# genome-vendor/allpathslg

Measured on NVIDIA B200. Metric: k-mer spectrum throughput (K=25), k-mer instances counted per second, higher is better.
Workload: dtype u64

## Files before the change

allpathslg_b200/csrc/local3.cuh:

```cuda
#pragma once
#include "local2.cuh"

#ifndef L3_PREFETCH
#define L3_PREFETCH 1
#endif
namespace apgk {

constexpr int L3_ROW = 16;
constexpr int L3_SLACK = 96;
constexpr int L3_STACK = 72;

struct Local3Smem {
  uint32_t* key; uint32_t* cnt; uint32_t* bitmap; uint16_t* list; uint32_t* spec; uint32_t* wsum; uint32_t* misc;
  uint32_t* stack;
  static __host__ __device__ size_t slots(int LM) { return (((size_t)LM + LM / 4 + 1 + L3_SLACK) + 127) & ~(size_t)127; }
  __device__ __forceinline__ void carve(unsigned char* raw, int LM) {
    const size_t ns = slots(LM);
    key = (uint32_t*)raw;
    cnt = key + ns;
    bitmap = cnt + ns;
    spec = bitmap + ns / 32 + 4;
    wsum = spec + SPEC_SMEM;
    misc = wsum + 40;
    stack = misc + 8;
    list = (uint16_t*)(stack + 2 * L3_STACK);
  }
  static size_t bytes(int LM) {
    return (slots(LM) * 2 + slots(LM) / 32 + 4 + SPEC_SMEM + 40 + 8 + 2 * L3_STACK) * 4 + ((size_t)LM + LM / 4 + 128) * 2 + 16;
  }
};

template <int NT, int W>
__global__ void __launch_bounds__(NT, 1536 / NT) k_local3(const uint32_t* __restrict__ src, BucketTable bt, int rem_bits, EmitCtx<W> ec,
                                               uint32_t* __restrict__ nd_out) {
  extern __shared__ __align__(16) unsigned char smem_raw[];
  Local3Smem sm;
  const int LM = (int)bt.local_max;
  sm.carve(smem_raw, LM);
  const int tid = threadIdx.x, lane = tid & 31, wid = tid >> 5;
  constexpr int NWARP = NT / 32;
  for (int i = tid; i < SPEC_SMEM; i += NT) sm.spec[i] = 0;
  const int up = 32 - rem_bits;
  const uint32_t m_cap = (uint32_t)LM + (uint32_t)LM / 4 + 1;
  unsigned long long n_nx = 0, o_nx = 0;
  if (bt.b0 + blockIdx.x < bt.nb) { n_nx = bt.bsize[bt.b0 + blockIdx.x]; o_nx = bt.bofs[bt.b0 + blockIdx.x]; }
  for (uint32_t b = bt.b0 + blockIdx.x; b < bt.nb; b += gridDim.x) {
    const unsigned long long n64 = n_nx;
    const unsigned long long o = o_nx;
    {
      const uint32_t bn = b + gridDim.x;
      if (bn < bt.nb) { n_nx = bt.bsize[bn]; o_nx = bt.bofs[bn]; }
    }
    if (n64 == 0) {
      if (tid == 0) nd_out[b] = 0;
      continue;
    }
    const uint32_t* s = src + o;
    const uint32_t m_want = n64 < (unsigned long long)LM ? (uint32_t)n64 + ((uint32_t)n64 >> 2) + 1 : m_cap;
    const uint32_t nrows = (m_want + L3_ROW - 1) / L3_ROW;
    const uint32_t ns = nrows * L3_ROW;
    const uint32_t ns4 = (ns + 3) >> 2;
    const uint32_t nwords = (ns + 31) >> 5;
    volatile uint32_t* vmisc = sm.misc;
    uint32_t run_nd = 0;
    bool first = true;
    while (true) {
      __syncthreads();
      uint32_t sp = 1, rd = 0, ri = 0;
      if (!first) {
        sp = sm.misc[1];
        if (sp == 0) break;
        rd = sm.stack[2 * (sp - 1)];
        ri = sm.stack[2 * (sp - 1) + 1];
      }
      first = false;
      {
        uint4* k4 = reinterpret_cast<uint4*>(sm.key);
        uint4* c4 = reinterpret_cast<uint4*>(sm.cnt);
        const uint4 e4 = make_uint4(SLOT_EMPTY, SLOT_EMPTY, SLOT_EMPTY, SLOT_EMPTY), z4 = make_uint4(0, 0, 0, 0);
        for (uint32_t i = tid; i < ns4; i += NT) { k4[i] = e4; c4[i] = z4; }
        for (uint32_t i = tid; i < nwords + 2; i += NT) sm.bitmap[i] = 0;
        if (tid == 0) sm.misc[0] = 0;
      }
      __syncthreads();
      if (tid == 0) sm.misc[1] = sp - 1;
      const uint32_t pshift = 32 - rd;
      for (unsigned long long i0 = 0; i0 < n64; i0 += 4ull * NT) {
        uint32_t kk[4];
#pragma unroll
        for (int u = 0; u < 4; u++) {
          const unsigned long long i = i0 + (unsigned long long)u * NT + tid;
          kk[u] = i < n64 ? s[i] : SLOT_EMPTY;
        }
#pragma unroll
        for (int u = 0; u < 4; u++) {
          const uint32_t k = kk[u];
          const uint32_t x = k << up;
          if (k != SLOT_EMPTY && (rd == 0 || (x >> pshift) == ri)) {
            const uint32_t row = __umulhi(x << rd, nrows) * L3_ROW;
            uint32_t h = (k * 0x9E3779B1u) >> 28;
            uint32_t slot = row + h;
            uint32_t cur = atomicCAS(&sm.key[slot], SLOT_EMPTY, k);
            if (cur == SLOT_EMPTY) atomicOr(&sm.bitmap[slot >> 5], 1u << (slot & 31));
            bool placed = (cur == SLOT_EMPTY) | (cur == k);
            for (int pr = 1; !placed; pr++) {
              if (pr == L3_ROW) { sm.misc[0] = 1u; break; }
              h = (h + 1) & (L3_ROW - 1);
              slot = row + h;
              cur = atomicCAS(&sm.key[slot], SLOT_EMPTY, k);
              if (cur == SLOT_EMPTY) atomicOr(&sm.bitmap[slot >> 5], 1u << (slot & 31));
              placed = (cur == SLOT_EMPTY) | (cur == k);
            }
            if (placed) atomicAdd(&sm.cnt[slot], 1u);
          }
          __syncwarp();
        }
        if (n64 > (unsigned long long)LM && __any_sync(0xffffffffu, vmisc[0] != 0)) break;
      }
      __syncthreads();
#if L3_PREFETCH
      if (L3_PREFETCH == 1 || run_nd == 0) {
        const unsigned long long i = (unsigned long long)tid * 32;
        if (b + gridDim.x < bt.nb && i < n_nx && tid < 1024) prefetch_l2(src + o_nx + i);
      }
#endif
      uint32_t nd_total;
      {
        constexpr int WPT = 2;
        uint32_t wd[WPT], c = 0;
#pragma unroll
        for (int u = 0; u < WPT; u++) {
          const uint32_t wi = tid * WPT + u;
          wd[u] = wi < nwords ? sm.bitmap[wi] : 0u;
          c += __popc(wd[u]);
        }
        const uint32_t incl = warp_incl_scan(c, lane);
        if (lane == 31) sm.wsum[wid] = incl;
        __syncthreads();
        uint32_t base = incl - c;
        nd_total = 0;
#pragma unroll
        for (int w = 0; w < NWARP; w++) {
          const uint32_t v = sm.wsum[w];
          if (w < wid) base += v;
          nd_total += v;
        }
        const bool failed = sm.misc[0] != 0;
        if (!failed) {
#pragma unroll
          for (int u = 0; u < WPT; u++) {
            uint32_t w = wd[u];
            const uint32_t s_base = (tid * WPT + u) << 5;
            while (w) {
              const int bit = __ffs((int)w) - 1;
              w &= w - 1;
              sm.list[base++] = (uint16_t)(s_base + bit);
            }
          }
        }
      }
      __syncthreads();
      if (sm.misc[0] != 0) {
        if (tid == 0) {
          uint32_t top = sm.misc[1];
          if ((int)rd < rem_bits && top + 2 <= L3_STACK) {
            sm.stack[2 * top] = rd + 1; sm.stack[2 * top + 1] = 2 * ri + 1; top++;
            sm.stack[2 * top] = rd + 1; sm.stack[2 * top + 1] = 2 * ri; top++;
            sm.misc[1] = top;
          } else {
            sm.misc[2] = 1u;
          }
        }
        continue;
      }
      for (uint32_t j0 = 0; j0 < nd_total; j0 += NT) {
        const uint32_t j = j0 + tid;
        uint32_t f = 0;
        if (j < nd_total) {
          const uint32_t q = sm.list[j];
          const uint32_t k = sm.key[q];
          const uint32_t rbase = q & ~(uint32_t)(L3_ROW - 1);
          uint32_t rowbits = (sm.bitmap[q >> 5] >> (rbase & 31)) & 0xFFFFu;
          const uint32_t before = __popc(rowbits & ((1u << (q & (L3_ROW - 1))) - 1u));
          uint32_t smaller = 0;
          while (rowbits) {
            const int bit = __ffs((int)rowbits) - 1;
            rowbits &= rowbits - 1;
            smaller += sm.key[rbase + bit] < k;
          }
          const unsigned long long pos = o + run_nd + (j - before + smaller);
          f = sm.cnt[q];
          if (ec.want_table) {
            ec.tmp_keys[pos] = rebuild_key<W>(k, (uint64_t)b, ec.rem_bits, ec.pad);
            ec.tmp_cnt[pos] = f;
          }
        }
        const uint32_t ones = __ballot_sync(0xffffffffu, f == 1u);
        if (lane == 0 && ones) atomicAdd(&sm.spec[1], (uint32_t)__popc(ones));
        if (f > 1u) {
          if (f < SPEC_SMEM) atomicAdd(&sm.spec[f], 1u);
          else spec_add_global(ec.spec_dense, ec.spec_ovf, ec.spec_ovf_cap, f);
        }
      }
      run_nd += nd_total;
      if (sm.misc[1] == 0) break;
    }
    if (tid == 0) nd_out[b] = run_nd;
  }
  __syncthreads();
  for (int i = tid; i < SPEC_SMEM; i += NT) {
    const uint32_t v = sm.spec[i];
    if (v) atomicAdd(&ec.spec_dense[i], (unsigned long long)v);
  }
}

}
```

allpathslg_b200/csrc/apgk.cu:

```cuda
#include <algorithm>
#include <array>
#include <cmath>
#include <cstdio>
#include <cstdlib>
#include <cstring>
#include <ctime>
#include <map>
#include <string>
#include <type_traits>
#include <utility>
#include <vector>

#include "../../include/apgk.h"
#include "gfreq.cuh"

using namespace apgk;

namespace {

enum Stage { ST_HIST0, ST_SCAN0, ST_SCATTER0, ST_HIST1, ST_SCAN1, ST_SCATTER1, ST_LOCAL, ST_BIG, ST_TABLE, ST_SPECTRUM,
             ST_OWNER, ST_TOTAL, ST_PLAN, ST_REDUCE };
const char* kStageNames[APGK_N_STAGES] = {"hist0", "scan0", "scatter0", "hist1", "scan1", "scatter1",
                                          "local", "big", "table", "spectrum", "owner", "total", "plan", "reduce"};

// ... 136 lines not shown
    c->ivs.push_back(iv);
  }
  apgk_ctx::StageIv& iv = c->ivs[c->n_ivs];
  iv.stage = s; iv.ended = false;
  c->open_iv[s] = (int)c->n_ivs++;
  if (kTrace) fprintf(stderr, "[apgk %.2f] begin %s\n", trace_now(), kStageNames[s]);
  cudaEventRecord(iv.e0, c->stream);
}
void stage_end(apgk_ctx* c, int s) {
  const int i = c->open_iv[s];
  if (i < 0) return;
  cudaEventRecord(c->ivs[i].e1, c->stream);
  c->ivs[i].ended = true;
  c->open_iv[s] = -1;
  if (kTrace) fprintf(stderr, "[apgk %.2f] end   %s\n", trace_now(), kStageNames[s]);
}
void stages_collect(apgk_ctx* c) {
  for (size_t i = 0; i < c->n_ivs; i++) {
    float ms = 0;
    if (c->ivs[i].ended && cudaEventElapsedTime(&ms, c->ivs[i].e0, c->ivs[i].e1) == cudaSuccess) c->stage_ms[c->ivs[i].stage] += ms;
  }
  c->n_ivs = 0;
}

int words_for(int K) { return (2 * K + 63) / 64; }

template <int W> struct Geo;
#ifndef APGK_NT
#define APGK_NT 1024
#endif
template <> struct Geo<1> { static constexpr int NTS = APGK_NT; static constexpr int NPOS = 16; static constexpr int NT0 = APGK_NT; static constexpr int NT1 = APGK_NT; static constexpr uint32_t TILE1 = APGK_NT * 16; static constexpr int LM_KEY = 4096; };
template <> struct Geo<2> { static constexpr int NTS = 1024; static constexpr int NPOS = 8; static constexpr int NT0 = 512; static constexpr int NT1 = 512; static constexpr uint32_t TILE1 = 512 * 8;  static constexpr int LM_KEY = 2048; };
template <> struct Geo<3> { static constexpr int NTS = 1024; static constexpr int NPOS = 4; static constexpr int NT0 = 256; static constexpr int NT1 = 512; static constexpr uint32_t TILE1 = 512 * 5;  static constexpr int LM_KEY = 2048; };
constexpr int LM_U32 = 5120;
constexpr int LM_KEY4 = 3072;
static bool use_local4(int W) {
  static const bool off = getenv("APGK_NO_LOCAL4") != nullptr;
  static const bool all = getenv("APGK_LOCAL4") != nullptr && !strcmp(getenv("APGK_LOCAL4"), "all");
  return !off && (W == 1 || all);
}
constexpr int L3_NT = 512;
constexpr int COL_NT = 1024;

void build_plan(HostPlan& hp, const std::vector<uint64_t>& seg_sizes, uint32_t tile_elems, int bins) {
  const int S = (int)seg_sizes.size();
  hp.seg_tile0.assign(S + 1, 0); hp.seg_chunk0.assign(S + 1, 0); hp.seg_start.assign(S + 1, 0);
  uint64_t max_tiles = 1;
  for (int s = 0; s < S; s++) {
    uint64_t t = (seg_sizes[s] + tile_elems - 1) / tile_elems;
    hp.seg_tile0[s + 1] = hp.seg_tile0[s] + (uint32_t)t;
    hp.seg_start[s + 1] = hp.seg_start[s] + seg_sizes[s];
    max_tiles = std::max(max_tiles, t);
  }
  int ct = (int)((max_tiles + 3) / 4);
  ct = std::max(8, std::min(ct, 128));
  if (const char* e = getenv("APGK_CT")) { if (atoi(e) > 0) ct = atoi(e); }
  for (int s = 0; s < S; s++) {
    uint32_t t = hp.seg_tile0[s + 1] - hp.seg_tile0[s];
    hp.seg_chunk0[s + 1] = hp.seg_chunk0[s] + (t + ct - 1) / ct;
  }
  hp.lp.bins = bins; hp.lp.n_segments = S; hp.lp.chunk_tiles = ct;
  hp.lp.n_tiles = hp.seg_tile0[S]; hp.lp.n_chunks = hp.seg_chunk0[S]; hp.lp.tile_elems = tile_elems;
}

int column_scan(apgk_ctx* c, const HostPlan& hp, int fold, unsigned long long* bofs_out) {
  const LevelPlan& lp = hp.lp;
  if (lp.n_chunks == 0) return APGK_OK;
  CU(c->segtot.ensure((size_t)lp.n_segments * lp.bins * 8));
  CU(c->bstart32.ensure((size_t)lp.n_segments * lp.bins * 4));
  k_segscan<COL_NT><<<lp.n_segments, COL_NT, 0, c->stream>>>(lp, c->chunksum.as<uint32_t>(),
                                                            c->segtot.as<unsigned long long>(),
                                                            c->bstart32.as<uint32_t>(), bofs_out, fold);
  LAUNCHED();
  return APGK_OK;
// ... 86 lines not shown
    const uint64_t sb_byte = src_bit0 >> 3;
    const uint64_t sb_al = sb_byte & ~7ull;
    const size_t nbytes = (size_t)(((src_bit0 + 2 * n_bases + 7) >> 3) - sb_al);
    CU(c->staging.ensure(nbytes + 32));
    CU(cudaMemsetAsync((uint8_t*)c->staging.p + (nbytes & ~(size_t)7), 0, 24, c->stream));
    CU(cudaMemcpyAsync(c->staging.p, packed + sb_al, nbytes, cudaMemcpyHostToDevice, c->stream));
    const uint64_t nbits = 2 * n_bases;
    const uint64_t nwords = ((dst_bit0 + nbits + 63) >> 6) - (dst_bit0 >> 6);
    k_append_bits<<<(unsigned)((nwords + 255) / 256), 256, 0, c->stream>>>(
        c->staging.as<uint64_t>(), src_bit0 - sb_al * 8, c->bases.as<uint64_t>(), dst_bit0, nbits);
    LAUNCHED();
  }
  return APGK_OK;
}

void invalidate_results(apgk_ctx* c) {
  c->finished = false; c->have_table = false; c->spec_loaded = false;
  c->table_from_reads = false; c->have_occ = false; c->n_occ = 0;
  c->n_instances = c->n_distinct = 0;
  c->owner_ranks = 0;
  c->part_ready = false; c->part_n = 0;
}

enum RunMode { RUN_FULL = 0, RUN_PARTITION = 1 };
template <int W, typename ElemB>
int run_levels(apgk_ctx* c, const Key<W>* dev_keys, uint64_t n_keys, RunMode mode);
template <int W, typename ElemB>
int count_buckets(apgk_ctx* c, uint64_t Nr, uint64_t N_all, uint64_t& n_prev, Key<W>* tmp_keys, bool nosync);

uint64_t window_upper(const apgk_ctx* c) { return c->n_windows; }

template <int W>
bool select_geometry(apgk_ctx* c, uint64_t upper, int forced_P) {
  int lm_u32 = LM_U32;
  if (const char* e = getenv("APGK_LM")) { if (atoi(e) >= 256 && atoi(e) <= 12288) lm_u32 = atoi(e); }
  if (upper == 0) upper = 1;
  if (forced_P > 0) {
    make_geom(c, std::max(2, std::min(24, forced_P)));
    return W == 1 && c->geom.REM <= 32;
  }
  int P = choose_prefix_bits(c, upper, lm_u32, true);
  make_geom(c, P);
  if (W == 1 && c->cfg.prefix_bits <= 0 && !getenv("APGK_PREFIX_BITS")) {
    while (c->geom.REM > 31 && c->geom.REM <= 34 && P < 24) make_geom(c, ++P);
  }
  const bool u32 = (W == 1 && c->geom.REM <= 32);
  if (!u32) {
    P = use_local4(W) ? choose_prefix_bits(c, upper, LM_KEY4 * 3 / 4, true) : choose_prefix_bits(c, upper, Geo<W>::LM_KEY, false);
    make_geom(c, P);
  }
  return u32;
}

template <int W> int compact_table(apgk_ctx* c, uint64_t total);

enum { RES_RANGE_N = 0, RES_SUM_TOT0 = 1, RES_FLAGS = 2, RES_DISTINCT = 3, RES_TABLE_OVF = 4, RES_XFLAGS = 5, RES_WORDS = 16 };

int fetch_results(apgk_ctx* c) {
  CU(cudaMemcpyAsync(c->res_host, c->res.p, RES_WORDS * 8, cudaMemcpyDeviceToHost, c->stream));
  CU(cudaStreamSynchronize(c->stream));
  return APGK_OK;
}

int step_epilogue(apgk_ctx* c, bool full) {
  { int r2 = fetch_results(c); if (r2) return r2; }
  if (c->res_host[RES_FLAGS] & 1ull) FAIL(APGK_E_RANGE, "a level-0 bucket holds 2^32 or more k-mers");
  if (c->res_host[RES_SUM_TOT0] && c->res_host[RES_SUM_TOT0] != c->n_windows_run)
    FAIL(APGK_E_STATE, "internal: level-0 histogram counts %llu k-mers, the input holds %llu",
         (unsigned long long)c->res_host[RES_SUM_TOT0], (unsigned long long)c->n_windows_run);
  if (full && c->table_pending) {
    c->table_pending = false;
    const uint64_t total = c->res_host[RES_DISTINCT];
    if (c->res_host[RES_TABLE_OVF]) {
      int rc = APGK_E_ARG;
// ... 252 lines not shown
    const char* eb = getenv("APGK_BULK");
    const bool bulk = eb && !strcmp(eb, "1");
    const size_t smb = scatter_bulk_smem_bytes<ElemB>(tile, bins1);
    if (bulk && sizeof(ElemB) == 4 && smb <= 200 * 1024 && bins1 <= Geo<W>::NT1) {
      auto kern = k_scatter_keys_bulk<Key<W>, ElemB, Geo<W>::NT1, DIGIT_BITS, false>;
      { int rc = kernel_setup(c, kern, Geo<W>::NT1, smb, nullptr); if (rc) return rc; }
      kern<<<chunks_bound, Geo<W>::NT1, smb, c->stream>>>(a_src, lp, dg1, c->chunksum.as<uint32_t>(), nullptr, g.pad, g.REM,
                                                          c->B.as<ElemB>());
    } else {
      auto kern = ScatterSel<ElemB, W>::kernel();
      const size_t sm = scatter_smem_bytes<Key<W>>(tile, bins1);
      { int rc = kernel_setup(c, kern, Geo<W>::NT1, sm, nullptr); if (rc) return rc; }
      kern<<<chunks_bound, Geo<W>::NT1, sm, c->stream>>>(a_src, lp, dg1, c->chunksum.as<uint32_t>(), nullptr, g.pad, g.REM,
                                                         c->B.as<ElemB>());
    }
    LAUNCHED();
  }
  stage_end(c, ST_SCATTER1);
  return APGK_OK;
}

int temp_budget(apgk_ctx* c, size_t* budget) {
  size_t fr = 0, tot = 0;
  CU(cudaMemGetInfo(&fr, &tot));
  const size_t held = c->A.cap + c->B.cap + c->T.cap;
  *budget = (size_t)((double)(fr + held) * 0.60);
  return APGK_OK;
}

template <int W, typename ElemB>
int run_levels(apgk_ctx* c, const Key<W>* dev_keys, uint64_t n_keys, RunMode mode) {
  const KeyGeom g = c->geom;
  const int bins0 = 1 << g.D0, bins1 = 1 << g.D1;
  int local_max = std::is_same<ElemB, uint32_t>::value ? LM_U32 : (use_local4(W) ? LM_KEY4 : Geo<W>::LM_KEY);
  if (std::is_same<ElemB, uint32_t>::value) {
    if (const char* e = getenv("APGK_LM")) { if (atoi(e) >= 256 && atoi(e) <= 12288) local_max = atoi(e); }
  }
  const int want_table = (c->cfg.flags & APGK_WANT_COUNTS) ? 1 : 0;
  c->elem_bytes = sizeof(ElemB);
  c->local_max = (uint32_t)local_max;
  c->nb1 = (uint32_t)bins0 * (uint32_t)bins1;
  c->n_rounds = 0; c->n_big = 0; c->n_distinct = 0;
  c->table_pending = false;
  CU(c->spec_dense.ensure((size_t)SPEC_DENSE * 8));
  CU(cudaMemsetAsync(c->spec_dense.p, 0, (size_t)SPEC_DENSE * 8, c->stream));
  CU(c->out_off.ensure(((size_t)c->nb1 + 1) * 8));
  CU(cudaMemsetAsync(c->out_off.p, 0, ((size_t)c->nb1 + 1) * 8, c->stream));
  const uint64_t N = dev_keys ? n_keys : c->n_windows;
  c->n_instances = N; c->n_windows_run = N;
  c->tot0_host.assign((size_t)bins0, 0);
  if (N == 0) {
    { int rc = wait_ingest(c); if (rc) return rc; }
    c->have_table = want_table != 0;
    c->part_n = 0;
    if (mode == RUN_PARTITION) {
      CU(c->segtot.ensure((size_t)c->nb1 * 8));
      CU(cudaMemsetAsync(c->segtot.p, 0, (size_t)c->nb1 * 8, c->stream));
    }
    return APGK_OK;
  }

  DigitSpec ds0{DIGIT_BITS, g.TB - g.D0, g.D0, g.pad, 0};
  DigitFn<DIGIT_BITS> dg0 = make_digit_fn<DIGIT_BITS>(ds0);
  { int rc = level0_hist<W>(c, dev_keys, n_keys, dg0); if (rc) return rc; }

  const size_t eA = sizeof(Key<W>), eB = sizeof(ElemB) + (want_table ? 4 : 0);
  uint64_t cap_outer = c->cfg.max_round_keys, cap_inner = c->cfg.max_inner_keys;
  if (const char* e = getenv("APGK_ROUND_KEYS")) { if (atoll(e) > 0) cap_outer = (uint64_t)atoll(e); }
  if (const char* e = getenv("APGK_INNER_KEYS")) { if (atoll(e) > 0) cap_inner = (uint64_t)atoll(e); }
  bool single;
// ... 91 lines not shown
      { int rc = level1<W, ElemB>(c, (int)in[0], (int)in[1], n_in, a_src, 0); if (rc) return rc; }
      if (mode == RUN_PARTITION) { c->part_n = n_in; return APGK_OK; }
      c->count_src = c->B.p; c->bucket_lo = c->bucket_hi = 0;
      if (!single) { c->bucket_lo = (uint32_t)in[0] * (uint32_t)bins1; c->bucket_hi = (uint32_t)in[1] * (uint32_t)bins1; }
      c->table_scale = single ? 1.0 : std::max(1.0, (double)N / (double)std::max<uint64_t>(n_counted, 1));
      { int rc = count_buckets<W, ElemB>(c, n_in, N, n_prev, a_src, single); if (rc) return rc; }
      c->table_scale = 1.0;
      c->bucket_lo = c->bucket_hi = 0;
      off_a += n_in;
    }
  }
  if (!single) c->n_distinct = n_prev;
  c->have_table = want_table != 0;
  return APGK_OK;
}

template <int W>
int compact_table(apgk_ctx* c, uint64_t total) {
  CU(c->out_keys.ensure(std::max<size_t>(total + (total >> 5), 1) * sizeof(Key<W>)));
  CU(c->out_cnt.ensure(std::max<size_t>(total + (total >> 5), 1) * 4));
  k_compact<W><<<c->n_sm * 8, 256, 0, c->stream>>>(c->tmp_keys_last ? (const Key<W>*)c->tmp_keys_last : c->A.as<Key<W>>(), c->T.as<uint32_t>(),
                                                   c->bofs.as<unsigned long long>(), c->out_off_local.as<unsigned long long>(), c->nb1,
                                                   c->out_keys.as<Key<W>>(), c->out_cnt.as<uint32_t>(), nullptr, 0ull, nullptr);
  LAUNCHED();
  return APGK_OK;
}

template <int W, typename ElemB>
int count_buckets(apgk_ctx* c, uint64_t Nr, uint64_t N, uint64_t& n_prev, Key<W>* tmp_keys, bool nosync) {
  const KeyGeom g = c->geom;
  const int local_max = (int)c->local_max;
  int l3_nt = L3_NT;
  if (std::is_same<ElemB, uint32_t>::value) {
    if (const char* e = getenv("APGK_L3_NT")) { if (atoi(e) == 256 || atoi(e) == 512) l3_nt = atoi(e); }
  }
  const bool use_l3 = std::is_same<ElemB, uint32_t>::value && g.REM >= 1 && g.REM <= 31;
  const bool use_l4 = !std::is_same<ElemB, uint32_t>::value && use_local4(W) && g.pad == 0 && g.REM >= 1;
  const int want_table = (c->cfg.flags & APGK_WANT_COUNTS) ? 1 : 0;
  const uint32_t big_cap = (uint32_t)(Nr / local_max + 16);
  uint64_t n_big = 0;
  unsigned long long stats[2] = {0, 0};
  if (!(use_l3 || use_l4)) {
    CU(c->big_list.ensure((size_t)big_cap * 4));
    CU(cudaMemsetAsync(c->stats.p, 0, 64, c->stream));
    k_classify<<<(c->nb1 + 255) / 256, 256, 0, c->stream>>>(c->segtot.as<unsigned long long>(), c->nb1, (uint32_t)local_max,
                                                           c->big_list.as<uint32_t>(), big_cap, c->stats.as<unsigned long long>());
    LAUNCHED();
    CU(cudaMemcpyAsync(stats, c->stats.p, 16, cudaMemcpyDeviceToHost, c->stream));
    CU(cudaStreamSynchronize(c->stream));
    n_big = stats[0];
    c->n_big += n_big;
  }
  {
    EmitCtx<W> ec;
    ec.want_table = want_table; ec.rem_bits = g.REM; ec.pad = g.pad;
    ec.tmp_keys = tmp_keys;
    c->tmp_keys_last = tmp_keys;
    if (want_table) CU(c->T.ensure(std::max<size_t>(Nr, 1) * 4));
    ec.tmp_cnt = c->T.as<uint32_t>();
    ec.spec_dense = c->spec_dense.as<unsigned long long>();
    ec.spec_ovf = c->spec_ovf.as<unsigned long long>();
    ec.spec_ovf_cap = (uint32_t)(N / SPEC_DENSE + 8);
    BucketTable bt;
    bt.bofs = c->bofs.as<unsigned long long>();
    bt.bsize = c->segtot.as<unsigned long long>();
    bt.nb = c->bucket_hi ? c->bucket_hi : c->nb1; bt.local_max = (uint32_t)local_max; bt.b0 = c->bucket_hi ? c->bucket_lo : 0;
    if (c->bucket_hi) CU(cudaMemsetAsync(c->nd.p, 0, ((size_t)c->nb1 + 1) * 4, c->stream));
    CU(c->deferred.ensure(((size_t)c->nb1 + 1) * 4));
    CU(cudaMemsetAsync(c->deferred.p, 0, 4, c->stream));
    stage_begin(c, ST_LOCAL);
    if (use_l3) {
      if constexpr (std::is_same<ElemB, uint32_t>::value) {
        auto launch3 = [&](auto kern3, int nt) -> int {
          const size_t sm3 = Local3Smem::bytes(local_max);
          int occ3 = 1;
          { int rc = kernel_setup(c, kern3, nt, sm3, &occ3); if (rc) return rc; }
          const uint32_t grid3 = std::min<uint32_t>(c->nb1, (uint32_t)(c->n_sm * std::max(occ3, 1)));
          kern3<<<grid3, nt, sm3, c->stream>>>((const uint32_t*)c->count_src, bt, g.REM, ec, c->nd.as<uint32_t>());
          return APGK_OK;
        };
        int rc3 = l3_nt == 256 ? launch3(k_local3<256, W>, 256) : launch3(k_local3<512, W>, 512);
        if (rc3) return rc3;
        LAUNCHED();
      }
    } else if (use_l4) {
      if constexpr (!std::is_same<ElemB, uint32_t>::value) {
        auto kern4 = k_local4<512, W>;
        const size_t sm4 = Local4Smem::bytes(local_max, W);
        int occ4 = 1;
        { int rc = kernel_setup(c, kern4, 512, sm4, &occ4); if (rc) return rc; }
        const uint32_t grid4 = std::min<uint32_t>(c->nb1, (uint32_t)(c->n_sm * std::max(occ4, 1)));
        kern4<<<grid4, 512, sm4, c->stream>>>((const Key<W>*)c->count_src, bt, g.REM, ec, c->nd.as<uint32_t>());
        LAUNCHED();
      }
    } else {
      auto kern2 = k_local2<ElemB, W>;
      const size_t sm2 = Local2Smem<ElemB>::bytes(local_max);
      int occ2 = 1;
      { int rc = kernel_setup(c, kern2, L2_NT, sm2, &occ2); if (rc) return rc; }
      const uint32_t grid2 = std::min<uint32_t>(c->nb1, (uint32_t)(c->n_sm * std::max(occ2, 1)));
      kern2<<<grid2, L2_NT, sm2, c->stream>>>((const ElemB*)c->count_src, bt, g.REM, ec, c->nd.as<uint32_t>(),
                                              c->deferred.as<uint32_t>(), c->nb1);
      LAUNCHED();
      auto kern = k_local<ElemB, W>;
      const size_t sm = LocalSmem<ElemB>::bytes(local_max);
      int occ = 1;
      { int rc = kernel_setup(c, kern, LOCAL_NT, sm, &occ); if (rc) return rc; }
      const uint32_t grid = std::min<uint32_t>(c->nb1, (uint32_t)(c->n_sm * std::max(occ, 1)));
      kern<<<grid, LOCAL_NT, sm, c->stream>>>((const ElemB*)c->count_src, bt, g.REM, ec, c->nd.as<uint32_t>(),
                                              c->deferred.as<uint32_t>(), c->nb1);
      LAUNCHED();
    }
    stage_end(c, ST_LOCAL);
    if (n_big) {
// ... 1436 lines not shown
  }
  return APGK_OK;
}

int apgk_debug_host_table_find(int K, const uint64_t* sorted_kmers, uint64_t n, int prefix_bits, const uint64_t* queries,
                               uint64_t n_q, uint64_t* idx_out) {
  if (K < 1 || K > APGK_MAX_K || prefix_bits < 1 || prefix_bits > 24) return APGK_E_ARG;
  if (words_for(K) > 1 && prefix_bits > 2 * K) return APGK_E_ARG;
  switch (words_for(K)) {
    case 1: host_table_find<1>(K, sorted_kmers, n, prefix_bits, queries, n_q, idx_out); break;
    case 2: host_table_find<2>(K, sorted_kmers, n, prefix_bits, queries, n_q, idx_out); break;
    case 3: host_table_find<3>(K, sorted_kmers, n, prefix_bits, queries, n_q, idx_out); break;
  }
  return APGK_OK;
}

int apgk_debug_host_splitters(const uint32_t* bucket_sizes, uint32_t n_buckets, uint32_t world, uint32_t bucket_cost, uint32_t* bounds_out) {
  if (!bucket_sizes || !bounds_out || !world) return APGK_E_ARG;
  std::vector<unsigned long long> S((size_t)n_buckets + 1, 0);
  for (uint32_t b = 0; b < n_buckets; b++) S[b + 1] = S[b] + (bucket_sizes[b] ? (unsigned long long)bucket_sizes[b] + bucket_cost : 0ull);
  for (uint32_t r = 0; r <= world; r++) bounds_out[r] = splitter_bound(S.data(), n_buckets, world, r);
  return APGK_OK;
}

int apgk_debug_host_synth(const apgk_synth_params* p, uint64_t r0, uint64_t n_reads, uint8_t* packed_out) {
  if (!p || !packed_out) return APGK_E_ARG;
  SynthParams sp{p->genome_len, p->seed_g, p->seed_p, p->seed_q, p->seed_r, p->seed_e, p->read_len, p->err_per_200};
  const uint64_t nb = n_reads * (uint64_t)p->read_len;
  uint32_t* w = (uint32_t*)packed_out;
  for (uint64_t wi = 0; wi * 16 < nb; wi++) w[wi] = synth_word(sp, r0, wi * 16, nb);
  return APGK_OK;
}

}
```

allpathslg_b200/csrc/group.cuh:

```cuda
#pragma once
#include <dlfcn.h>
#include <nccl.h>

namespace {

struct NcclApi {
  void* h = nullptr;
  ncclResult_t (*GetUniqueId)(ncclUniqueId*) = nullptr;
  ncclResult_t (*CommInitRank)(ncclComm_t*, int, ncclUniqueId, int) = nullptr;
  ncclResult_t (*CommDestroy)(ncclComm_t) = nullptr;
  ncclResult_t (*AllGather)(const void*, void*, size_t, ncclDataType_t, ncclComm_t, cudaStream_t) = nullptr;
  ncclResult_t (*AllReduce)(const void*, void*, size_t, ncclDataType_t, ncclRedOp_t, ncclComm_t, cudaStream_t) = nullptr;
  const char* (*GetErrorString)(ncclResult_t) = nullptr;
  std::string load() {
    if (h) return "";
    for (const char* name : {"libnccl.so.2", "libnccl.so"}) {
      h = dlopen(name, RTLD_NOW | RTLD_GLOBAL);
      if (h) break;
    }
    if (!h) return std::string("cannot load libnccl.so.2: ") + dlerror();
    auto sym = [&](const char* n) { return dlsym(h, n); };
    GetUniqueId = (decltype(GetUniqueId))sym("ncclGetUniqueId");
    CommInitRank = (decltype(CommInitRank))sym("ncclCommInitRank");
    CommDestroy = (decltype(CommDestroy))sym("ncclCommDestroy");
// ... 263 lines not shown
    r.host = nullptr; r.host_words = 0;
    if (r.ev_a) cudaEventDestroy(r.ev_a);
    if (r.ev_b) cudaEventDestroy(r.ev_b);
    r.ev_a = r.ev_b = nullptr;
    r.c = nullptr;
    c->group = nullptr;
    g->dead = true;
  }
}

struct HostLayout {
  size_t plan = 0, extra = 0, red = 0, ovf = 0, tot0 = 0, words = 0;
  HostLayout(int world, int bins0) {
    plan = 0;
    extra = plan + 3 * ((size_t)world + 1);
    red = extra + 4;
    ovf = red + SPEC_DENSE + 2;
    tot0 = ovf + (size_t)world * (1 + OVF_SHIP);
    words = tot0 + 2 * (size_t)bins0;
  }
};

struct GRound { int lo, hi; std::vector<std::array<int, 2>> inner; };

template <int W, typename ElemB>
int group_count_typed(apgk_group* g, const std::vector<GroupMeta>& meta, bool single, uint64_t cap_outer, uint64_t cap_inner, int d2,
                      uint64_t budget, double inner_bytes) {
  const int world = g->world, nl = g->n_local;
  apgk_ctx* c0 = g->rs[0].c;
  const KeyGeom gp = c0->geom;
  const int bins0 = 1 << gp.D0, bins1 = 1 << gp.D1;
  const uint32_t nb = (uint32_t)bins0 * (uint32_t)bins1, nbf = nb << d2;
  const int want_table = (c0->cfg.flags & APGK_WANT_COUNTS) ? 1 : 0;
  int local_max = std::is_same<ElemB, uint32_t>::value ? LM_U32 : (use_local4(W) ? LM_KEY4 : Geo<W>::LM_KEY);
  if (std::is_same<ElemB, uint32_t>::value) {
    if (const char* e = getenv("APGK_LM")) { if (atoi(e) >= 256 && atoi(e) <= 12288) local_max = atoi(e); }
  }
  uint32_t bucket_cost = std::is_same<ElemB, uint32_t>::value ? 800u : 0u;
  if (const char* e = getenv("APGK_BUCKET_COST")) bucket_cost = (uint32_t)std::max(0, atoi(e));
  if (world == 1) bucket_cost = 0;
  const HostLayout hl(world, bins0);
  uint64_t N_sum = 0, N_max = 0;
  for (int s = 0; s < world; s++) { N_sum += meta[s].n_windows; N_max = std::max<uint64_t>(N_max, meta[s].n_windows); }

  for (RankState& r : g->rs) {
    apgk_ctx* c = r.c;
    GCU(cudaSetDevice(c->device));
    invalidate_results(c);
    stages_reset(c);
    if (!c->res_host) GCU(cudaHostAlloc((void**)&c->res_host, RES_WORDS * 8, cudaHostAllocDefault));
    GCU(c->res.ensure(RES_WORDS * 8));
    GCU(cudaMemsetAsync(c->res.p, 0, RES_WORDS * 8, c->stream));
    if (r.host_words < hl.words) {
      if (r.host) cudaFreeHost(r.host);
      r.host = nullptr; r.host_words = 0;
      GCU(cudaHostAlloc((void**)&r.host, hl.words * 8, cudaHostAllocDefault));
      r.host_words = hl.words;
    }
    r.geom_part = gp;
    r.geom_shard = gp; r.geom_shard.D1 += d2; r.geom_shard.REM -= d2;
    r.nb = nb; r.nbf = nbf;
    r.n_prev = 0; r.shard_n = 0; r.remote_bytes = 0;
    c->geom = gp;
    c->elem_bytes = sizeof(ElemB);
    c->local_max = (uint32_t)local_max;
    c->nb1 = nb;
    c->n_rounds = 0; c->n_big = 0; c->n_distinct = 0; c->n_instances = 0;
    c->table_pending = false;
    c->n_windows_run = c->n_windows;
    stage_begin(c, ST_TOTAL);
// ... 619 lines not shown
```

Before: 48.82.

## Software-pipeline bucket key loads and clear only touched hash slots

Replaces the L2 prefetch with register-level software pipelining. Each thread loads the next batch of keys, including the first batch of the next bucket, before the current batch is processed. It also zeroes the whole shared hash table once at kernel start. Before each bucket pass it resets only the slots listed in the previous occupancy list, instead of clearing ns entries with vector stores. This aims to hide global load latency and cut per-bucket clearing cost, at the price of more live registers. It also depends on the list being correct even for failed passes, which is why the list is now always written.

```diff
diff --git a/allpathslg_b200/csrc/local3.cuh b/allpathslg_b200/csrc/local3.cuh
--- a/allpathslg_b200/csrc/local3.cuh
+++ b/allpathslg_b200/csrc/local3.cuh
@@ -1,9 +1,6 @@
 #pragma once
 #include "local2.cuh"
 
-#ifndef L3_PREFETCH
-#define L3_PREFETCH 1
-#endif
 namespace apgk {
 
 constexpr int L3_ROW = 16;
@@ -30,6 +27,16 @@
   }
 };
 
+template <int NT>
+__device__ __forceinline__ void l3_load_batch(uint32_t (&kk)[4], const uint32_t* __restrict__ s, unsigned long long n,
+                                              unsigned long long i0, int tid) {
+#pragma unroll
+  for (int u = 0; u < 4; u++) {
+    const unsigned long long i = i0 + (unsigned long long)u * NT + tid;
+    kk[u] = i < n ? s[i] : SLOT_EMPTY;
+  }
+}
+
 template <int NT, int W>
 __global__ void __launch_bounds__(NT, 1536 / NT) k_local3(const uint32_t* __restrict__ src, BucketTable bt, int rem_bits, EmitCtx<W> ec,
                                                uint32_t* __restrict__ nd_out) {
@@ -40,26 +47,31 @@
   const int tid = threadIdx.x, lane = tid & 31, wid = tid >> 5;
   constexpr int NWARP = NT / 32;
   for (int i = tid; i < SPEC_SMEM; i += NT) sm.spec[i] = 0;
+  for (uint32_t i = tid; i < (uint32_t)Local3Smem::slots(LM); i += NT) { sm.key[i] = SLOT_EMPTY; sm.cnt[i] = 0; }
+  uint32_t nd_used = 0;
   const int up = 32 - rem_bits;
   const uint32_t m_cap = (uint32_t)LM + (uint32_t)LM / 4 + 1;
   unsigned long long n_nx = 0, o_nx = 0;
   if (bt.b0 + blockIdx.x < bt.nb) { n_nx = bt.bsize[bt.b0 + blockIdx.x]; o_nx = bt.bofs[bt.b0 + blockIdx.x]; }
+  uint32_t kk[4];
+  l3_load_batch<NT>(kk, src + o_nx, n_nx, 0, tid);
   for (uint32_t b = bt.b0 + blockIdx.x; b < bt.nb; b += gridDim.x) {
     const unsigned long long n64 = n_nx;
     const unsigned long long o = o_nx;
     {
       const uint32_t bn = b + gridDim.x;
+      n_nx = 0; o_nx = 0;
       if (bn < bt.nb) { n_nx = bt.bsize[bn]; o_nx = bt.bofs[bn]; }
     }
     if (n64 == 0) {
       if (tid == 0) nd_out[b] = 0;
+      l3_load_batch<NT>(kk, src + o_nx, n_nx, 0, tid);
       continue;
     }
     const uint32_t* s = src + o;
     const uint32_t m_want = n64 < (unsigned long long)LM ? (uint32_t)n64 + ((uint32_t)n64 >> 2) + 1 : m_cap;
     const uint32_t nrows = (m_want + L3_ROW - 1) / L3_ROW;
     const uint32_t ns = nrows * L3_ROW;
-    const uint32_t ns4 = (ns + 3) >> 2;
     const uint32_t nwords = (ns + 31) >> 5;
     volatile uint32_t* vmisc = sm.misc;
     uint32_t run_nd = 0;
@@ -72,13 +84,15 @@
         if (sp == 0) break;
         rd = sm.stack[2 * (sp - 1)];
         ri = sm.stack[2 * (sp - 1) + 1];
+        l3_load_batch<NT>(kk, s, n64, 0, tid);
       }
       first = false;
       {
-        uint4* k4 = reinterpret_cast<uint4*>(sm.key);
-        uint4* c4 = reinterpret_cast<uint4*>(sm.cnt);
-        const uint4 e4 = make_uint4(SLOT_EMPTY, SLOT_EMPTY, SLOT_EMPTY, SLOT_EMPTY), z4 = make_uint4(0, 0, 0, 0);
-        for (uint32_t i = tid; i < ns4; i += NT) { k4[i] = e4; c4[i] = z4; }
+        for (uint32_t j = tid; j < nd_used; j += NT) {
+          const uint32_t q = sm.list[j];
+          sm.key[q] = SLOT_EMPTY;
+          sm.cnt[q] = 0;
+        }
         for (uint32_t i = tid; i < nwords + 2; i += NT) sm.bitmap[i] = 0;
         if (tid == 0) sm.misc[0] = 0;
       }
@@ -86,15 +100,13 @@
       if (tid == 0) sm.misc[1] = sp - 1;
       const uint32_t pshift = 32 - rd;
       for (unsigned long long i0 = 0; i0 < n64; i0 += 4ull * NT) {
-        uint32_t kk[4];
-#pragma unroll
-        for (int u = 0; u < 4; u++) {
-          const unsigned long long i = i0 + (unsigned long long)u * NT + tid;
-          kk[u] = i < n64 ? s[i] : SLOT_EMPTY;
-        }
 #pragma unroll
         for (int u = 0; u < 4; u++) {
           const uint32_t k = kk[u];
+          {
+            const unsigned long long i = i0 + (unsigned long long)(4 + u) * NT + tid;
+            kk[u] = i < n64 ? s[i] : SLOT_EMPTY;
+          }
           const uint32_t x = k << up;
           if (k != SLOT_EMPTY && (rd == 0 || (x >> pshift) == ri)) {
             const uint32_t row = __umulhi(x << rd, nrows) * L3_ROW;
@@ -118,12 +130,6 @@
         if (n64 > (unsigned long long)LM && __any_sync(0xffffffffu, vmisc[0] != 0)) break;
       }
       __syncthreads();
-#if L3_PREFETCH
-      if (L3_PREFETCH == 1 || run_nd == 0) {
-        const unsigned long long i = (unsigned long long)tid * 32;
-        if (b + gridDim.x < bt.nb && i < n_nx && tid < 1024) prefetch_l2(src + o_nx + i);
-      }
-#endif
       uint32_t nd_total;
       {
         constexpr int WPT = 2;
@@ -145,21 +151,20 @@
           if (w < wid) base += v;
           nd_total += v;
         }
-        const bool failed = sm.misc[0] != 0;
-        if (!failed) {
-#pragma unroll
-          for (int u = 0; u < WPT; u++) {
-            uint32_t w = wd[u];
-            const uint32_t s_base = (tid * WPT + u) << 5;
-            while (w) {
-              const int bit = __ffs((int)w) - 1;
-              w &= w - 1;
-              sm.list[base++] = (uint16_t)(s_base + bit);
-            }
-          }
-        }
-      }
-      __syncthreads();
+#pragma unroll
+        for (int u = 0; u < WPT; u++) {
+          uint32_t w = wd[u];
+          const uint32_t s_base = (tid * WPT + u) << 5;
+          while (w) {
+            const int bit = __ffs((int)w) - 1;
+            w &= w - 1;
+            sm.list[base++] = (uint16_t)(s_base + bit);
+          }
+        }
+      }
+      nd_used = nd_total;
+      __syncthreads();
+      l3_load_batch<NT>(kk, src + o_nx, n_nx, 0, tid);
       if (sm.misc[0] != 0) {
         if (tid == 0) {
           uint32_t top = sm.misc[1];
```

Measured after the change: 49.04, median of 6. No clear change (+0.4%).

## Decouple L3 bucket sizing from hash capacity and shrink shared-memory table

Applied to the files above, without the earlier changes.

Geometry selection still targets buckets of about 5120 keys, but the shared-memory hash table in the local3 kernel is now capped at 2048 slots instead of being sized to 1.25x the bucket limit. The kernel defaults to 256 threads and can grow to 512 when the slot count is large. Buckets that overflow the capped table fall back to the existing radix-split stack path. The aim is lower shared-memory use per CTA so more CTAs fit per SM, at the cost of more split passes on large buckets. L2 prefetch of the next bucket now covers up to 16K elements, and opt-in clock64 profiling instrumentation is added.

```diff
diff --git a/allpathslg_b200/csrc/apgk.cu b/allpathslg_b200/csrc/apgk.cu
--- a/allpathslg_b200/csrc/apgk.cu
+++ b/allpathslg_b200/csrc/apgk.cu
@@ -192,14 +192,19 @@
 template <> struct Geo<1> { static constexpr int NTS = APGK_NT; static constexpr int NPOS = 16; static constexpr int NT0 = APGK_NT; static constexpr int NT1 = APGK_NT; static constexpr uint32_t TILE1 = APGK_NT * 16; static constexpr int LM_KEY = 4096; };
 template <> struct Geo<2> { static constexpr int NTS = 1024; static constexpr int NPOS = 8; static constexpr int NT0 = 512; static constexpr int NT1 = 512; static constexpr uint32_t TILE1 = 512 * 8;  static constexpr int LM_KEY = 2048; };
 template <> struct Geo<3> { static constexpr int NTS = 1024; static constexpr int NPOS = 4; static constexpr int NT0 = 256; static constexpr int NT1 = 512; static constexpr uint32_t TILE1 = 512 * 5;  static constexpr int LM_KEY = 2048; };
-constexpr int LM_U32 = 5120;
+constexpr int L3_BUCKET_KEYS = 5120;
+constexpr int L3_CAP_SLOTS = 2048;
 constexpr int LM_KEY4 = 3072;
 static bool use_local4(int W) {
   static const bool off = getenv("APGK_NO_LOCAL4") != nullptr;
   static const bool all = getenv("APGK_LOCAL4") != nullptr && !strcmp(getenv("APGK_LOCAL4"), "all");
   return !off && (W == 1 || all);
 }
-constexpr int L3_NT = 512;
+constexpr int L3_NT = 256;
+static int l3_cap_slots() {
+  if (const char* e = getenv("APGK_L3_SLOTS")) { if (atoi(e) >= 256 && atoi(e) <= 32768) return atoi(e); }
+  return L3_CAP_SLOTS;
+}
 constexpr int COL_NT = 1024;
 
 void build_plan(HostPlan& hp, const std::vector<uint64_t>& seg_sizes, uint32_t tile_elems, int bins) {
@@ -352,14 +357,12 @@
 
 template <int W>
 bool select_geometry(apgk_ctx* c, uint64_t upper, int forced_P) {
-  int lm_u32 = LM_U32;
-  if (const char* e = getenv("APGK_LM")) { if (atoi(e) >= 256 && atoi(e) <= 12288) lm_u32 = atoi(e); }
   if (upper == 0) upper = 1;
   if (forced_P > 0) {
     make_geom(c, std::max(2, std::min(24, forced_P)));
     return W == 1 && c->geom.REM <= 32;
   }
-  int P = choose_prefix_bits(c, upper, lm_u32, true);
+  int P = choose_prefix_bits(c, upper, L3_BUCKET_KEYS, true);
   make_geom(c, P);
   if (W == 1 && c->cfg.prefix_bits <= 0 && !getenv("APGK_PREFIX_BITS")) {
     while (c->geom.REM > 31 && c->geom.REM <= 34 && P < 24) make_geom(c, ++P);
@@ -678,10 +681,7 @@
 int run_levels(apgk_ctx* c, const Key<W>* dev_keys, uint64_t n_keys, RunMode mode) {
   const KeyGeom g = c->geom;
   const int bins0 = 1 << g.D0, bins1 = 1 << g.D1;
-  int local_max = std::is_same<ElemB, uint32_t>::value ? LM_U32 : (use_local4(W) ? LM_KEY4 : Geo<W>::LM_KEY);
-  if (std::is_same<ElemB, uint32_t>::value) {
-    if (const char* e = getenv("APGK_LM")) { if (atoi(e) >= 256 && atoi(e) <= 12288) local_max = atoi(e); }
-  }
+  const int local_max = std::is_same<ElemB, uint32_t>::value ? l3_cap_slots() : (use_local4(W) ? LM_KEY4 : Geo<W>::LM_KEY);
   const int want_table = (c->cfg.flags & APGK_WANT_COUNTS) ? 1 : 0;
   c->elem_bytes = sizeof(ElemB);
   c->local_max = (uint32_t)local_max;
@@ -839,7 +839,8 @@
   const int local_max = (int)c->local_max;
   int l3_nt = L3_NT;
   if (std::is_same<ElemB, uint32_t>::value) {
-    if (const char* e = getenv("APGK_L3_NT")) { if (atoi(e) == 256 || atoi(e) == 512) l3_nt = atoi(e); }
+    if (const char* e = getenv("APGK_L3_NT")) { if (atoi(e) == 128 || atoi(e) == 256 || atoi(e) == 512) l3_nt = atoi(e); }
+    while (l3_nt < 512 && local_max > 64 * l3_nt) l3_nt *= 2;
   }
   const bool use_l3 = std::is_same<ElemB, uint32_t>::value && g.REM >= 1 && g.REM <= 31;
   const bool use_l4 = !std::is_same<ElemB, uint32_t>::value && use_local4(W) && g.pad == 0 && g.REM >= 1;
@@ -886,7 +887,8 @@
           kern3<<<grid3, nt, sm3, c->stream>>>((const uint32_t*)c->count_src, bt, g.REM, ec, c->nd.as<uint32_t>());
           return APGK_OK;
         };
-        int rc3 = l3_nt == 256 ? launch3(k_local3<256, W>, 256) : launch3(k_local3<512, W>, 512);
+        int rc3 = l3_nt == 128 ? launch3(k_local3<128, W>, 128)
+                  : l3_nt == 256 ? launch3(k_local3<256, W>, 256) : launch3(k_local3<512, W>, 512);
         if (rc3) return rc3;
         LAUNCHED();
       }
@@ -2389,4 +2391,17 @@
   return APGK_OK;
 }
 
-}
+#if APGK_L3_PROFILE
+int apgk_l3_profile_read(uint64_t* out16, int reset) {
+  if (!out16) return APGK_E_ARG;
+  if (cudaDeviceSynchronize() != cudaSuccess) return APGK_E_CUDA;
+  if (cudaMemcpyFromSymbol(out16, g_l3_prof, L3P_N * 8) != cudaSuccess) return APGK_E_CUDA;
+  if (reset) {
+    const unsigned long long z[L3P_N] = {};
+    if (cudaMemcpyToSymbol(g_l3_prof, z, sizeof z) != cudaSuccess) return APGK_E_CUDA;
+  }
+  return APGK_OK;
+}
+#endif
+
+}
diff --git a/allpathslg_b200/csrc/group.cuh b/allpathslg_b200/csrc/group.cuh
--- a/allpathslg_b200/csrc/group.cuh
+++ b/allpathslg_b200/csrc/group.cuh
@@ -319,10 +319,7 @@
   const int bins0 = 1 << gp.D0, bins1 = 1 << gp.D1;
   const uint32_t nb = (uint32_t)bins0 * (uint32_t)bins1, nbf = nb << d2;
   const int want_table = (c0->cfg.flags & APGK_WANT_COUNTS) ? 1 : 0;
-  int local_max = std::is_same<ElemB, uint32_t>::value ? LM_U32 : (use_local4(W) ? LM_KEY4 : Geo<W>::LM_KEY);
-  if (std::is_same<ElemB, uint32_t>::value) {
-    if (const char* e = getenv("APGK_LM")) { if (atoi(e) >= 256 && atoi(e) <= 12288) local_max = atoi(e); }
-  }
+  const int local_max = std::is_same<ElemB, uint32_t>::value ? l3_cap_slots() : (use_local4(W) ? LM_KEY4 : Geo<W>::LM_KEY);
   uint32_t bucket_cost = std::is_same<ElemB, uint32_t>::value ? 800u : 0u;
   if (const char* e = getenv("APGK_BUCKET_COST")) bucket_cost = (uint32_t)std::max(0, atoi(e));
   if (world == 1) bucket_cost = 0;
diff --git a/allpathslg_b200/csrc/local3.cuh b/allpathslg_b200/csrc/local3.cuh
--- a/allpathslg_b200/csrc/local3.cuh
+++ b/allpathslg_b200/csrc/local3.cuh
@@ -4,7 +4,36 @@
 #ifndef L3_PREFETCH
 #define L3_PREFETCH 1
 #endif
+#ifndef APGK_L3_PROFILE
+#define APGK_L3_PROFILE 0
+#endif
 namespace apgk {
+
+#if APGK_L3_PROFILE
+enum {
+  L3P_BAR_TOP = 0,
+  L3P_CLEAR, L3P_BAR_CLEAR, L3P_INSERT, L3P_BAR_INSERT, L3P_LIST, L3P_BAR_LIST, L3P_EMIT, L3P_TAIL,
+  L3P_TOTAL,
+  L3P_PASSES, L3P_FAILED, L3P_BUCKETS, L3P_EMPTY, L3P_CTAS,
+  L3P_N = 16
+};
+__device__ unsigned long long g_l3_prof[L3P_N];
+#define L3_MARK(ph)                                   \
+  do {                                                \
+    if (threadIdx.x == 0) {                           \
+      const long long t_ = clock64();                 \
+      l3p[ph] += (unsigned long long)(t_ - l3_t);     \
+      l3_t = t_;                                      \
+    }                                                 \
+  } while (0)
+#define L3_COUNT(ix) \
+  do {               \
+    if (threadIdx.x == 0) l3p[ix]++; \
+  } while (0)
+#else
+#define L3_MARK(ph) do { } while (0)
+#define L3_COUNT(ix) do { } while (0)
+#endif
 
 constexpr int L3_ROW = 16;
 constexpr int L3_SLACK = 96;
@@ -13,9 +42,9 @@
 struct Local3Smem {
   uint32_t* key; uint32_t* cnt; uint32_t* bitmap; uint16_t* list; uint32_t* spec; uint32_t* wsum; uint32_t* misc;
   uint32_t* stack;
-  static __host__ __device__ size_t slots(int LM) { return (((size_t)LM + LM / 4 + 1 + L3_SLACK) + 127) & ~(size_t)127; }
-  __device__ __forceinline__ void carve(unsigned char* raw, int LM) {
-    const size_t ns = slots(LM);
+  static __host__ __device__ size_t slots(int cap) { return ((size_t)cap + L3_SLACK + 127) & ~(size_t)127; }
+  __device__ __forceinline__ void carve(unsigned char* raw, int cap) {
+    const size_t ns = slots(cap);
     key = (uint32_t*)raw;
     cnt = key + ns;
     bitmap = cnt + ns;
@@ -25,8 +54,8 @@
     stack = misc + 8;
     list = (uint16_t*)(stack + 2 * L3_STACK);
   }
-  static size_t bytes(int LM) {
-    return (slots(LM) * 2 + slots(LM) / 32 + 4 + SPEC_SMEM + 40 + 8 + 2 * L3_STACK) * 4 + ((size_t)LM + LM / 4 + 128) * 2 + 16;
+  static size_t bytes(int cap) {
+    return (slots(cap) * 2 + slots(cap) / 32 + 4 + SPEC_SMEM + 40 + 8 + 2 * L3_STACK) * 4 + slots(cap) * 2 + 16;
   }
 };
 
@@ -35,13 +64,18 @@
                                                uint32_t* __restrict__ nd_out) {
   extern __shared__ __align__(16) unsigned char smem_raw[];
   Local3Smem sm;
-  const int LM = (int)bt.local_max;
-  sm.carve(smem_raw, LM);
+  const uint32_t cap = bt.local_max;
+  sm.carve(smem_raw, (int)cap);
   const int tid = threadIdx.x, lane = tid & 31, wid = tid >> 5;
   constexpr int NWARP = NT / 32;
   for (int i = tid; i < SPEC_SMEM; i += NT) sm.spec[i] = 0;
+#if APGK_L3_PROFILE
+  __shared__ unsigned long long l3p[L3P_N];
+  if (tid == 0) for (int i = 0; i < L3P_N; i++) l3p[i] = 0;
+  const long long l3_t0 = clock64();
+  long long l3_t = l3_t0;
+#endif
   const int up = 32 - rem_bits;
-  const uint32_t m_cap = (uint32_t)LM + (uint32_t)LM / 4 + 1;
   unsigned long long n_nx = 0, o_nx = 0;
   if (bt.b0 + blockIdx.x < bt.nb) { n_nx = bt.bsize[bt.b0 + blockIdx.x]; o_nx = bt.bofs[bt.b0 + blockIdx.x]; }
   for (uint32_t b = bt.b0 + blockIdx.x; b < bt.nb; b += gridDim.x) {
@@ -53,10 +87,14 @@
     }
     if (n64 == 0) {
       if (tid == 0) nd_out[b] = 0;
+      L3_COUNT(L3P_EMPTY);
       continue;
     }
+    L3_COUNT(L3P_BUCKETS);
     const uint32_t* s = src + o;
-    const uint32_t m_want = n64 < (unsigned long long)LM ? (uint32_t)n64 + ((uint32_t)n64 >> 2) + 1 : m_cap;
+    const unsigned long long want = n64 + (n64 >> 2) + 1;
+    const bool capped = want >= (unsigned long long)cap;
+    const uint32_t m_want = capped ? cap : (uint32_t)want;
     const uint32_t nrows = (m_want + L3_ROW - 1) / L3_ROW;
     const uint32_t ns = nrows * L3_ROW;
     const uint32_t ns4 = (ns + 3) >> 2;
@@ -74,6 +112,8 @@
         ri = sm.stack[2 * (sp - 1) + 1];
       }
       first = false;
+      L3_MARK(L3P_BAR_TOP);
+      L3_COUNT(L3P_PASSES);
       {
         uint4* k4 = reinterpret_cast<uint4*>(sm.key);
         uint4* c4 = reinterpret_cast<uint4*>(sm.cnt);
@@ -82,7 +122,9 @@
         for (uint32_t i = tid; i < nwords + 2; i += NT) sm.bitmap[i] = 0;
         if (tid == 0) sm.misc[0] = 0;
       }
-      __syncthreads();
+      L3_MARK(L3P_CLEAR);
+      __syncthreads();
+      L3_MARK(L3P_BAR_CLEAR);
       if (tid == 0) sm.misc[1] = sp - 1;
       const uint32_t pshift = 32 - rd;
       for (unsigned long long i0 = 0; i0 < n64; i0 += 4ull * NT) {
@@ -115,13 +157,15 @@
           }
           __syncwarp();
         }
-        if (n64 > (unsigned long long)LM && __any_sync(0xffffffffu, vmisc[0] != 0)) break;
-      }
-      __syncthreads();
+        if (capped && __any_sync(0xffffffffu, vmisc[0] != 0)) break;
+      }
+      L3_MARK(L3P_INSERT);
+      __syncthreads();
+      L3_MARK(L3P_BAR_INSERT);
 #if L3_PREFETCH
       if (L3_PREFETCH == 1 || run_nd == 0) {
-        const unsigned long long i = (unsigned long long)tid * 32;
-        if (b + gridDim.x < bt.nb && i < n_nx && tid < 1024) prefetch_l2(src + o_nx + i);
+        if (b + gridDim.x < bt.nb)
+          for (unsigned long long i = (unsigned long long)tid * 32; i < n_nx && i < 16384; i += 32 * NT) prefetch_l2(src + o_nx + i);
       }
 #endif
       uint32_t nd_total;
@@ -159,8 +203,11 @@
           }
         }
       }
-      __syncthreads();
+      L3_MARK(L3P_LIST);
+      __syncthreads();
+      L3_MARK(L3P_BAR_LIST);
       if (sm.misc[0] != 0) {
+        L3_COUNT(L3P_FAILED);
         if (tid == 0) {
           uint32_t top = sm.misc[1];
           if ((int)rd < rem_bits && top + 2 <= L3_STACK) {
@@ -203,6 +250,7 @@
         }
       }
       run_nd += nd_total;
+      L3_MARK(L3P_EMIT);
       if (sm.misc[1] == 0) break;
     }
     if (tid == 0) nd_out[b] = run_nd;
@@ -212,6 +260,14 @@
     const uint32_t v = sm.spec[i];
     if (v) atomicAdd(&ec.spec_dense[i], (unsigned long long)v);
   }
+#if APGK_L3_PROFILE
+  L3_MARK(L3P_TAIL);
+  if (tid == 0) {
+    l3p[L3P_TOTAL] = (unsigned long long)(clock64() - l3_t0);
+    l3p[L3P_CTAS] = 1;
+    for (int i = 0; i < L3P_N; i++) atomicAdd(&g_l3_prof[i], l3p[i]);
+  }
+#endif
 }
 
 }
```

New measurement: 48.85 before, 36.20 after (median of 6 runs). -25.9%, worse.
